# akvas/grates

Measured on AMD Instinct MI355X. Metric: d/o-96 solutions/s to 0.25deg grid + full-cov GFLOP/s at 1/2/4/8 MI355X, higher is better.
Workload: dtype f64; 1 GPU; batch of 240 monthly solutions d/o 96 -> 0.25 deg GeographicGrid (720x1440), kernel ewh, per GPU; max_degree=96, epochs_per_gpu=240, parallelism=epochs sharded over 1 GPU(s), no collective, fused_kernel=True, fourfold_symmetry=True, rotation_folded_kernel=True, rotations=10, settle_launches=300

## Files before the change

### grates_amd/_lib.py

```python

import ctypes
import os

_HERE = os.path.dirname(os.path.abspath(__file__))
LIB_PATH = os.path.join(_HERE, 'lib', 'libshg.so')

c_double_p = ctypes.c_void_p
c_plan_p = ctypes.c_void_p


class ShgError(RuntimeError):

    def __init__(self, function, status, message):
        super().__init__('{0} failed with status {1}: {2}'.format(function, status, message))
        self.function = function
        self.status = status


_POINTS_AT_TAIL = [ctypes.c_void_p, ctypes.c_void_p, ctypes.c_int, c_double_p, ctypes.c_int, ctypes.c_double, ctypes.c_double, c_double_p,
                   ctypes.c_void_p]

PROTOTYPES = {
    'shg_plan_create': [ctypes.POINTER(c_plan_p), ctypes.c_int, ctypes.c_int, c_double_p, c_double_p, ctypes.c_int, c_double_p, ctypes.c_int],
    'shg_plan_destroy': [c_plan_p],
    'shg_plan_set_chunk': [c_plan_p, ctypes.c_int],
    'shg_plan_set_path': [c_plan_p, ctypes.c_int],
    'shg_plan_set_rotations': [c_plan_p, ctypes.c_int],
    'shg_plan_set_stage_limit': [c_plan_p, ctypes.c_int],
    'shg_plan_set_order_pruning': [c_plan_p, ctypes.c_int],
    'shg_plan_order_cutoffs': [c_plan_p, ctypes.POINTER(ctypes.c_int), ctypes.c_int, ctypes.POINTER(ctypes.c_int), ctypes.POINTER(ctypes.c_int)],
    'shg_rot_order_cutoffs': [ctypes.c_int, ctypes.c_int, c_double_p, c_double_p, ctypes.POINTER(ctypes.c_int), ctypes.c_int, ctypes.POINTER(ctypes.c_int)],
    'shg_rot_level_tables': [ctypes.c_int, ctypes.c_int, ctypes.c_int, ctypes.c_int, ctypes.c_int, c_double_p, ctypes.POINTER(ctypes.c_int32), c_double_p,
                             ctypes.c_int64, ctypes.POINTER(ctypes.c_int32), ctypes.c_int64],
    'shg_plan_info': [c_plan_p, ctypes.POINTER(ctypes.c_int64)],
    'shg_analysis_info': [c_plan_p, c_double_p],
    'shg_plan_profile': [c_plan_p, ctypes.c_int],
    'shg_plan_profile_read': [c_plan_p, ctypes.POINTER(ctypes.c_double), ctypes.POINTER(ctypes.c_int64)],
    'shg_synthesis': [c_plan_p, c_double_p, ctypes.c_int, c_double_p, ctypes.c_void_p],
    'shg_synthesis_points': [ctypes.c_int, c_double_p, c_double_p, c_double_p, ctypes.c_int, c_double_p, ctypes.c_int, c_double_p, ctypes.c_void_p],
    'shg_legendre': [ctypes.c_int, c_double_p, ctypes.c_int, c_double_p, ctypes.c_void_p],
    'shg_legendre_order': [ctypes.c_int, ctypes.c_int, c_double_p, ctypes.c_int, c_double_p, ctypes.c_void_p],
    'shg_trigonometric': [ctypes.c_int, c_double_p, ctypes.c_int, c_double_p, ctypes.c_void_p],
    'shg_synthesis_matrix_order': [ctypes.c_int, ctypes.c_int, ctypes.c_int, c_double_p, ctypes.c_int, c_double_p, ctypes.c_int, c_double_p, ctypes.c_int,
                                   c_double_p, c_double_p, ctypes.c_void_p],
# ... 166 lines not shown
```

### grates_amd/csrc/common.h

```cpp
#pragma once

#include <hip/hip_runtime.h>

#include <algorithm>
#include <atomic>
#include <cstdarg>
#include <cstdint>
#include <cstdio>
#include <cstdlib>
#include <mutex>
#include <vector>

#include "../../include/shg.h"

namespace shg {

typedef double double4_t __attribute__((ext_vector_type(4)));

int fail(int code, const char* fmt, ...);
unsigned hip_failures();
int zero_fill(double* p, long long ld, long long cols, long long rows, hipStream_t stream);
int zero_fill(int* p, hipStream_t stream);
int triangle_copy(int n, const double* src, int ld, long long stride, int batch, double* dst, bool upper, hipStream_t stream);
enum ScratchSlot { kScratchSplitK = 0, kScratchAnaFold = 1, kScratchAnaTransform = 2, kScratchAnaSolution = 3, kScratchAnaFlag = 4,
// ... 210 lines not shown
constexpr int kRotPruneMaxDegree = 128;
constexpr int kEpochTile = 8;
constexpr int kLatTile = 64;

}

struct shg_plan {
    int device = 0;
    int N = 0, nlat = 0, nlon = 0;
    int ldlat = 0;
    bool sym4 = false;
    int rotR = 0;
    std::vector<double> lon_host;
    shg::DeviceArray<double> rot_trig;
    bool order_pruning = true;
    std::vector<int> rot_levels;
    std::vector<int> rot_level_set;
    std::vector<int> rot_trig_piece;
    std::vector<int> rot_item_rec, rot_item_nrec, rot_item_ntrip;
    shg::DeviceArray<int> rot_levtab_d;
    bool rot_levtab_valid = false;
    bool sym_ns = false;
    int ngroups = 1;
    int goff[5] = {0, 0, 0, 0, 0};
    int K = 0;
    int ncol = 0;
    int ncoltiles = 0;
    int chunk = 16;

    shg::DeviceArray<double> ct;
// ... 71 lines not shown
namespace shg {
int plan_alloc_workspace(shg_plan* p);
int fused_chunk_for(const shg_plan* p);
int build_pk_table(shg_plan* p, hipStream_t stream);
int build_pkf_table(shg_plan* p, bool ns, int rotR, hipStream_t stream);
int build_blockmap(shg_plan* p, int nbt, int nit, hipStream_t stream);
int pack_coefficients_fused(shg_plan* p, bool ns, int rotR, const double* anm, int B, hipStream_t stream);
int synthesis_fused(shg_plan* p, const double* anm, int B, double* grid, hipStream_t stream);
bool has_rotation_symmetry(int nlon, const double* lon, int R);
int rot_layout(int R, int N, int nk[kRotMaxClasses], int cnt[kRotMaxClasses], std::vector<int>* order_slot);
int rot_choose(int nlon, const double* lon_h, int N);
int rot_applicable(const shg_plan* p);
int build_rot_trig(shg_plan* p, const double* lon_h);
void rot_order_cutoffs(int N, int nlat, const double* colat, const double* kn, bool ns, std::vector<int>& levels);
std::vector<int> rot_level_list(int N, const std::vector<int>& levels);
void rot_trig_stream(int R, int N, int level, int nlon, const double* lon_h, std::vector<double>& tab);
void item_table_host(const shg_plan* p, int N, int level, int od, const std::vector<int>& qoff, int rotR, std::vector<int>& table, int& nrec, int& ntrip);
int synthesis_rot(shg_plan* p, const double* anm, int B, double* grid, hipStream_t stream);
int rot_kernel_waves();
int rot_set_stage_limit(shg_plan* p, int limit);
int fused32_applicable(const shg_plan* p);
int synthesis_fused32(shg_plan* p, const double* anm, int B, double* grid, hipStream_t stream);

struct PlanGuard {
    shg_plan* p;
    std::unique_lock<std::mutex> lock;
    PlanGuard(shg_plan* plan, hipStream_t stream) : p(plan), lock(plan->mtx) {
        if (p->used && p->last_stream != stream) {
            bool ordered = false;
            if (p->order_event || hipEventCreateWithFlags(&p->order_event, hipEventDisableTiming) == hipSuccess)
                ordered = hipEventRecord(p->order_event, p->last_stream) == hipSuccess && hipStreamWaitEvent(stream, p->order_event, 0) == hipSuccess;
// ... 19 lines not shown
```

### grates_amd/csrc/plan.hip

```cpp
#include <atomic>
#include <cmath>
#include <cstring>
#include <string>

#include <map>
#include <memory>
#include <mutex>
#include <utility>
#include <vector>

#include "common.h"

namespace shg {

static thread_local std::string g_last_error;
static std::atomic<unsigned> g_hip_failures{0};

int fail(int code, const char* fmt, ...) {
    char buf[512];
    va_list ap;
    va_start(ap, fmt);
    vsnprintf(buf, sizeof(buf), fmt, ap);
    va_end(ap);
    g_last_error = buf;
// ... 483 lines not shown

extern "C" int shg_plan_set_stage_limit(shg_plan* p, int limit) {
    SHG_REQUIRE(p != nullptr, "shg_plan_set_stage_limit: NULL plan");
    std::unique_lock<std::mutex> lock(p->mtx);
    return rot_set_stage_limit(p, limit);
}

extern "C" int shg_plan_set_order_pruning(shg_plan* p, int enable) {
    SHG_REQUIRE(p != nullptr, "shg_plan_set_order_pruning: NULL plan");
    SHG_REQUIRE(enable == 0 || enable == 1, "shg_plan_set_order_pruning: %d not in {0, 1}", enable);
    std::unique_lock<std::mutex> lock(p->mtx);
    p->order_pruning = enable != 0;
    return SHG_OK;
}

extern "C" int shg_plan_order_cutoffs(const shg_plan* p, int* levels, int capacity, int* nblocks, int* enabled) {
    SHG_REQUIRE(p != nullptr && nblocks != nullptr, "shg_plan_order_cutoffs: NULL argument");
    SHG_REQUIRE(capacity >= 0 && (levels != nullptr || capacity == 0), "shg_plan_order_cutoffs: NULL table of %d entries", capacity);
    const bool applies = rot_applicable(p) && !p->rot_levels.empty();
    *nblocks = applies ? (int)p->rot_levels.size() : 0;
    if (enabled) *enabled = applies && p->order_pruning ? 1 : 0;
    for (int i = 0; i < *nblocks && i < capacity; ++i) levels[i] = p->rot_levels[i];
    return SHG_OK;
}

extern "C" int shg_rot_order_cutoffs(int N, int nlat, const double* colat_h, const double* kn_h, int* levels, int capacity, int* nblocks) {
    SHG_REQUIRE(N >= 1 && N <= kRotPruneMaxDegree, "shg_rot_order_cutoffs: degree %d out of range [1, %d]", N, kRotPruneMaxDegree);
    SHG_REQUIRE(nlat > 0 && colat_h && kn_h && nblocks, "shg_rot_order_cutoffs: NULL or empty table");
    SHG_REQUIRE(capacity >= 0 && (levels != nullptr || capacity == 0), "shg_rot_order_cutoffs: NULL table of %d entries", capacity);
    std::vector<int> badmap, lv;
// ... 9 lines not shown
extern "C" int shg_rot_level_tables(int R, int N, int level, int ns, int nlon, const double* lon_h, int32_t header[24], double* trig, int64_t trig_capacity,
                                    int32_t* items, int64_t items_capacity) {
    SHG_REQUIRE(R == 3 || R == 6 || R == 9 || R == 10, "shg_rot_level_tables: %d rotations not in {3, 6, 9, 10}", R);
    SHG_REQUIRE(N >= 1 && N <= kRotPruneMaxDegree && level >= 1 && level <= N, "shg_rot_level_tables: level %d of degree %d out of range", level, N);
    SHG_REQUIRE(nlon >= 2 * R && nlon % (2 * R) == 0 && lon_h && header, "shg_rot_level_tables: NULL table or nlon %d no multiple of %d", nlon, 2 * R);
    SHG_REQUIRE(trig_capacity >= 0 && items_capacity >= 0 && (trig || trig_capacity == 0) && (items || items_capacity == 0), "shg_rot_level_tables: NULL table");
    for (int i = 0; i < kRotLevelInts; ++i) header[i] = 0;
    int nk[kRotMaxClasses], cnt[kRotMaxClasses];
    header[1] = rot_layout(R, level, nk, cnt, nullptr);
    header[0] = header[1] / 4;
    for (int c = 0; c < kRotMaxClasses; ++c) {
        header[8 + c] = nk[c];
        header[8 + kRotMaxClasses + c] = cnt[c];
    }
    std::vector<double> tab;
    rot_trig_stream(R, N, level, nlon, lon_h, tab);
    const int od = ns ? 16 : 8;
    std::vector<int> qoff(N + 2), table;
    int q = 0;
    for (int m = 0; m <= N; ++m) {
        qoff[m] = q;
        q += (N + 1 - m + od - 1) / od;
    }
    qoff[N + 1] = q;
    int nrec = 0, ntrip = 0;
    item_table_host(nullptr, N, level, od, qoff, R, table, nrec, ntrip);
    header[2] = nrec;
    header[3] = ntrip;
    header[4] = (int32_t)(tab.size() / 128);
    header[5] = (int32_t)(table.size() / 4);
    for (size_t i = 0; i < tab.size() && (int64_t)i < trig_capacity; ++i) trig[i] = tab[i];
// ... 15 lines not shown
        return fail(SHG_ERR_UNSUPPORTED, "shg_plan_set_rotations: the panel of %d rotations at degree %d does not fit the LDS", want, p->N);
    }
    SHG_HIP(hipDeviceSynchronize());
    if (rot_applicable(p)) {
        const int rc = build_rot_trig(p, p->lon_host.data());
        if (rc) return rc;
    }
    return SHG_OK;
}

extern "C" int shg_plan_info(const shg_plan* p, int64_t which[8]) {
    SHG_REQUIRE(p != nullptr && which != nullptr, "shg_plan_info: NULL argument");
    which[0] = p->N;
    which[1] = p->nlat;
    which[2] = p->nlon;
    which[3] = (p->sym4 ? 1 : 0) | (p->sym_ns ? 2 : 0) | (rot_applicable(p) ? 4 : 0);
    which[4] = p->chunk;
    which[5] = p->K;
    which[6] = (p->path >= 2 || (p->path == 0 && (rot_applicable(p) || fused_chunk_for(p) != 0 || fused32_applicable(p)))) ? 1 : 0;
    which[7] = p->path | (rot_applicable(p) ? p->rotR << 8 : 0);
    return SHG_OK;
}
```

### grates_amd/csrc/synthesis_rot.hip

```cpp
#include <algorithm>
#include <cmath>
#include <cstdlib>

#include "common.h"

#ifndef SHG_STORE_AUX
#define SHG_STORE_AUX 2
#endif

namespace shg {

typedef double double2_t __attribute__((ext_vector_type(2)));
typedef unsigned int uint4_t __attribute__((ext_vector_type(4)));

#ifndef SHG_ROT_PREFERENCE
#define SHG_ROT_PREFERENCE 10, 9, 6, 3
#endif
#ifndef SHG_ROT_WAVES
#define SHG_ROT_WAVES 8
#endif
#ifndef SHG_RING_DEPTH
#define SHG_RING_DEPTH (SHG_ROT_WAVES > 8 ? 3 : 5)
#endif
constexpr int kWaves = SHG_ROT_WAVES;
constexpr int kColStride = kWaves / 4;
constexpr int kRingDepth = SHG_RING_DEPTH;
constexpr int kRingSlots = kRingDepth + 1;
constexpr int kRingDoubles = kWaves * kRingSlots * 128;
constexpr int kMaxClasses = kRotMaxClasses;

template <int R>
struct RotTraits {
    static constexpr int kClasses = R / 2 + 1, kTwo = R % 2 == 0 ? 2 : 1, kAcc = 2 * R;
    static constexpr int acc_of(int r) { return r == 0 ? 0 : (R % 2 == 0 && 2 * r == R) ? 2 : 2 * kTwo + 4 * (r - 1); }
};

struct RotParams {
    int N, nlat, nlon, B, nit, nh;
    int nd;
    int nct;
    int npieces;
    int cls_nk[kMaxClasses];
    int cls_cnt[kMaxClasses];
    int nslot;
#ifdef SHG_EXPERIMENT
    int dbg;
    int stagger;
    int stagger2;
#endif
    int Qtot;
    const double* cpk4;
    const double* pkf;
    const int4* itemtab;
    int nrec, ntrip;
    int* tickets;
// ... 37 lines not shown

__device__ __forceinline__ void store_b64_soff(double v, int4_s rsrc, unsigned voff, unsigned soff) {
    asm volatile("s_mov_b32 m0, %3\n\ts_nop 0\n\tbuffer_store_dwordx2 %0, %1, %2, m0 offen nt"
                 :
                 : "v"(v), "v"(voff), "s"(rsrc), "s"(soff)
                 : "memory");
}

template <int N>
__device__ __forceinline__ void wait_vmcnt() {
    asm volatile("s_waitcnt vmcnt(%0)" ::"i"(N) : "memory");
    __builtin_amdgcn_sched_barrier(0);
}

template <int R>
__device__ __forceinline__ void rot_images(double4_t* acc, int r);

template <>
__device__ __forceinline__ void rot_images<6>(double4_t* acc, int r) {
    constexpr double g = 0.86602540378443864676;
    const double ca0 = acc[0][r], sb0 = acc[1][r], ca3 = acc[2][r], sb3 = acc[3][r];
    const double ca1 = acc[4][r], sa1 = acc[5][r], cb1 = acc[6][r], sb1 = acc[7][r];
    const double ca2 = acc[8][r], sa2 = acc[9][r], cb2 = acc[10][r], sb2 = acc[11][r];
#pragma unroll
    for (int sgn = 0; sgn < 2; ++sgn) {
        const double x0 = sgn ? ca0 - sb0 : ca0 + sb0, x3 = sgn ? ca3 - sb3 : ca3 + sb3;
        const double x1 = sgn ? ca1 - sb1 : ca1 + sb1, y1 = sgn ? cb1 + sa1 : cb1 - sa1;
        const double x2 = sgn ? ca2 - sb2 : ca2 + sb2, y2 = sgn ? cb2 + sa2 : cb2 - sa2;
        const double t = fma(-0.5, x2, x0);
        const double e0 = x0 + x2, e1 = fma(g, y2, t), e2 = fma(-g, y2, t);
        const double u = fma(0.5, x1, -x3);
        const double o0 = x1 + x3, o1 = fma(g, y1, u), o2 = fma(g, y1, -u);
        acc[6 * sgn + 0][r] = e0 + o0;
        acc[6 * sgn + 3][r] = e0 - o0;
        acc[6 * sgn + 1][r] = e1 + o1;
        acc[6 * sgn + 4][r] = e1 - o1;
        acc[6 * sgn + 2][r] = e2 + o2;
        acc[6 * sgn + 5][r] = e2 - o2;
    }
}

template <>
__device__ __forceinline__ void rot_images<3>(double4_t* acc, int r) {
    constexpr double g = 0.86602540378443864676;
    const double ca0 = acc[0][r], sb0 = acc[1][r];
    const double ca1 = acc[2][r], sa1 = acc[3][r], cb1 = acc[4][r], sb1 = acc[5][r];
#pragma unroll
    for (int sgn = 0; sgn < 2; ++sgn) {
        const double x0 = sgn ? ca0 - sb0 : ca0 + sb0;
        const double x1 = sgn ? ca1 - sb1 : ca1 + sb1, y1 = sgn ? cb1 + sa1 : cb1 - sa1;
        const double t = fma(-0.5, x1, x0);
        acc[3 * sgn + 0][r] = x0 + x1;
        acc[3 * sgn + 1][r] = fma(g, y1, t);
        acc[3 * sgn + 2][r] = fma(-g, y1, t);
    }
}

template <>
__device__ __forceinline__ void rot_images<9>(double4_t* acc, int r) {
    constexpr double c1 = 0.76604444311897803520, c2 = 0.17364817766693034885, c4 = -0.93969262078590838405;
    constexpr double s1 = 0.64278760968653932632, s2 = 0.98480775301220805937, s3 = 0.86602540378443864676, s4 = 0.34202014332566873304;
    const double ca0 = acc[0][r], sb0 = acc[1][r];
    double ca[4], sa[4], cb[4], sb[4];
#pragma unroll
    for (int j = 0; j < 4; ++j) {
        ca[j] = acc[2 + 4 * j][r];
        sa[j] = acc[3 + 4 * j][r];
        cb[j] = acc[4 + 4 * j][r];
        sb[j] = acc[5 + 4 * j][r];
    }
#pragma unroll
    for (int sgn = 0; sgn < 2; ++sgn) {
        const double x0 = sgn ? ca0 - sb0 : ca0 + sb0;
        double x[4], y[4];
#pragma unroll
        for (int j = 0; j < 4; ++j) {
            x[j] = sgn ? ca[j] - sb[j] : ca[j] + sb[j];
            y[j] = sgn ? cb[j] + sa[j] : cb[j] - sa[j];
        }
        const double x1 = x[0], x2 = x[1], x3 = x[2], x4 = x[3], y1 = y[0], y2 = y[1], y3 = y[2], y4 = y[3];
        const double t = (x1 + x2) + x4, x03 = x0 + x3;
        const double h = fma(-0.5, x3, x0), u = s3 * y3;
        const double C1 = fma(c1, x1, fma(c2, x2, fma(c4, x4, h)));
        const double C2 = fma(c2, x1, fma(c4, x2, fma(c1, x4, h)));
        const double C3 = fma(-0.5, t, x03);
        const double C4 = fma(c4, x1, fma(c1, x2, fma(c2, x4, h)));
        const double S1 = fma(s1, y1, fma(s2, y2, fma(s4, y4, u)));
        const double S2 = fma(s2, y1, fma(s4, y2, fma(-s1, y4, -u)));
        const double S3 = s3 * ((y1 - y2) + y4);
        const double S4 = fma(s4, y1, fma(-s1, y2, fma(-s2, y4, u)));
        acc[9 * sgn + 0][r] = x03 + t;
        acc[9 * sgn + 1][r] = C1 + S1;
        acc[9 * sgn + 8][r] = C1 - S1;
        acc[9 * sgn + 2][r] = C2 + S2;
        acc[9 * sgn + 7][r] = C2 - S2;
        acc[9 * sgn + 3][r] = C3 + S3;
        acc[9 * sgn + 6][r] = C3 - S3;
        acc[9 * sgn + 4][r] = C4 + S4;
        acc[9 * sgn + 5][r] = C4 - S4;
    }
}

template <>
__device__ __forceinline__ void rot_images<10>(double4_t* acc, int r) {
    constexpr double c1 = 0.80901699437494742410, c2 = 0.30901699437494742410;
    constexpr double s1 = 0.58778525229247312917, s2 = 0.95105651629515357212;
    const double ca0 = acc[0][r], sb0 = acc[1][r], ca5 = acc[2][r], sb5 = acc[3][r];
    double ca[4], sa[4], cb[4], sb[4];
#pragma unroll
    for (int j = 0; j < 4; ++j) {
        ca[j] = acc[4 + 4 * j][r];
        sa[j] = acc[5 + 4 * j][r];
        cb[j] = acc[6 + 4 * j][r];
        sb[j] = acc[7 + 4 * j][r];
    }
#pragma unroll
    for (int sgn = 0; sgn < 2; ++sgn) {
        const double x0 = sgn ? ca0 - sb0 : ca0 + sb0, x5 = sgn ? ca5 - sb5 : ca5 + sb5;
        double x[4], y[4];
#pragma unroll
        for (int j = 0; j < 4; ++j) {
            x[j] = sgn ? ca[j] - sb[j] : ca[j] + sb[j];
            y[j] = sgn ? cb[j] + sa[j] : cb[j] - sa[j];
        }
        const double x1 = x[0], x2 = x[1], x3 = x[2], x4 = x[3], y1 = y[0], y2 = y[1], y3 = y[2], y4 = y[3];
        const double e0 = (x0 + x2) + x4;
        const double a1 = fma(c2, x2, fma(-c1, x4, x0)), b1 = fma(s2, y2, s1 * y4);
        const double a2 = fma(-c1, x2, fma(c2, x4, x0)), b2 = fma(s1, y2, -(s2 * y4));
        const double e1 = a1 + b1, e4 = a1 - b1, e2 = a2 + b2, e3 = a2 - b2;
        const double o0 = (x1 + x3) + x5;
        const double p = fma(c1, x1, fma(-c2, x3, -x5)), q = fma(s1, y1, s2 * y3);
        const double u = fma(c2, x1, fma(-c1, x3, x5)), v = fma(s2, y1, -(s1 * y3));
        const double o1 = q + p, o4 = q - p, o2 = v + u, o3 = v - u;
        acc[10 * sgn + 0][r] = e0 + o0;
        acc[10 * sgn + 5][r] = e0 - o0;
        acc[10 * sgn + 1][r] = e1 + o1;
        acc[10 * sgn + 6][r] = e1 - o1;
        acc[10 * sgn + 2][r] = e2 + o2;
        acc[10 * sgn + 7][r] = e2 - o2;
        acc[10 * sgn + 3][r] = e3 + o3;
        acc[10 * sgn + 8][r] = e3 - o3;
        acc[10 * sgn + 4][r] = e4 + o4;
        acc[10 * sgn + 9][r] = e4 - o4;
    }
}

struct RotStream {
    const double* iptr;
    const double* ibase;
    const double* ifirst;
    const double* ilast;
    int irem;
    unsigned im0, ring_lds;
    int cslot, pf;
    double2_t tx, abx;
};

constexpr int EP = 4;
__device__ __forceinline__ void rot_stream_init(RotStream& S, const RotParams& P, const double* As, int wave) {
// ... 19 lines not shown
    return;
#endif
    S.im0 = S.im0 + 1024 == S.ring_lds + kRingSlots * 1024 ? S.ring_lds : S.im0 + 1024;
    const bool more = S.irem > 1;
    const double* nbase = S.ibase == S.ilast ? S.ifirst : S.ibase + kColStride * P.npieces * 128;
    S.ibase = more ? S.ibase : nbase;
    S.iptr = more ? S.iptr + 128 : nbase;
    S.irem = more ? S.irem - 1 : P.npieces;
}

template <bool NS, int R>
__device__ __forceinline__ void rot_phase2(const RotParams& P, const double* As, const double2_t* panel, RotStream& S, int wave, int lane,
                                           int b0, int it) {
    constexpr int PR = 16 * EP;
    using T = RotTraits<R>;
    constexpr int kImages = 2 * R;
    const int fr = lane & 15, fk = lane >> 4;
    const int i0 = it * 16, i0n = it * 8;
    const unsigned lane_off = (unsigned)lane * 16u;
    auto grid_row = [&](int s) { return NS ? (s < 8 ? i0n + s : P.nlat - 1 - (i0n + s - 8)) : i0 + s; };
    auto slot_valid = [&](int s) { return NS ? i0n + (s & 7) < P.nh : i0 + s < P.nlat; };

    const int grid_bytes = P.nlat * P.nlon * 8;
    const int n2 = P.nlon >> 1, nR = P.nlon / R;
    const double2_t* const ringp = reinterpret_cast<const double2_t*>(As) + wave * (kRingSlots * 64) + lane;
    const int rt = wave % EP;
    const double2_t* const prow = panel + rt * 16 + fr + fk * PR;
#define ROT_FETCH(T_, AB_)                                                                                \
    do {                                                                                                  \
        __builtin_amdgcn_sched_barrier(0);                                                                \
        if (!(SHG_ROT_X & 8)) rot_issue_piece(S, P, lane_off);                                            \
// ... 73 lines not shown
        {
            const double2_t* z = panel + P.nslot * PR + rt * 16 + fk;
#pragma unroll
            for (int r = 0; r < 4; ++r) acc[0][r] = z[4 * r].x;
        }
#pragma unroll
        for (int c = 0; c < T::kClasses; ++c) {
            if (c < T::kTwo) {
                ROT_CLASS(c, ROT_MFMA2, 2 * c, 2)
            } else {
                ROT_CLASS(c, ROT_MFMA4, 2 * T::kTwo + 4 * (c - T::kTwo), 4)
            }
        }
        ROT_STAMP(3 + 2 * min(q, 3));

#pragma unroll
        for (int r = 0; r < 4; ++r) rot_images<R>(acc, r);
        const int b = b0 + rt;
        const bool epoch_ok = b < P.B && !SHG_DBG(P, 1);
        double* const Gb = P.G + (size_t)min(b, P.B - 1) * P.nlat * P.nlon;
        {
            const __amdgpu_buffer_rsrc_t rsrc = __builtin_amdgcn_make_buffer_rsrc(Gb, 0, grid_bytes, 0x00020000);
            const int par = fr & 1, ce = fr & ~1;
            const int sa = fk + (par ? 8 : 0), sb = sa + 4;
            const bool col_ok = epoch_ok && ct * 16 + ce < P.nd;
            const unsigned row_a = col_ok && slot_valid(sa) ? (unsigned)grid_row(sa) * (unsigned)P.nlon * 8u : 0x80000000u;
            const unsigned row_b = col_ok && slot_valid(sb) ? (unsigned)grid_row(sb) * (unsigned)P.nlon * 8u : 0x80000000u;
            const unsigned asc = (unsigned)ce * 8u, desc = (unsigned)(14 - ce) * 8u;
#pragma unroll
            for (int t = 0; t < kImages; ++t) {
                const int k = t < R ? t : t - R;
                const bool ascending = t < R;
                int w = n2 + k * nR - (ascending ? 0 : P.nd);
                w = w >= P.nlon ? w - P.nlon : w;
                const int soff = (ascending ? w + 16 * ct : w + P.nd - 16 * ct - 16) * 8;
                double a_lo, a_hi, b_lo, b_hi;
                pair_exchange(acc[t][0], acc[t][2], 0xAAAAAAAAAAAAAAAAull, a_lo, a_hi);
                pair_exchange(acc[t][1], acc[t][3], 0xAAAAAAAAAAAAAAAAull, b_lo, b_hi);
                const double2_t va = ascending ? (double2_t){a_lo, a_hi} : (double2_t){a_hi, a_lo};
                const double2_t vb = ascending ? (double2_t){b_lo, b_hi} : (double2_t){b_hi, b_lo};
                const unsigned lane_col = (ascending ? asc : desc) + (unsigned)soff;
                __builtin_amdgcn_raw_buffer_store_b128(__builtin_bit_cast(uint4_t, va), rsrc, row_a + lane_col, 0, SHG_STORE_AUX);
                __builtin_amdgcn_raw_buffer_store_b128(__builtin_bit_cast(uint4_t, vb), rsrc, row_b + lane_col, 0, SHG_STORE_AUX);
            }
        }
        ROT_STAMP(4 + 2 * min(q, 3));
    }
    S.tx = tx;
    S.abx = abx;
#undef ROT_CLASS
#undef ROT_MFMA2
#undef ROT_MFMA4
#undef ROT_MFMA2_FIRST
#undef ROT_MFMA4_FIRST
#undef ROT_FETCH
}

__device__ __forceinline__ void panel_put(double2_t* panel, int index, double2_t v) { panel[index] = v; }
// ... 202 lines not shown
    if (P.stagger2 > 0 && wave >= EP) {
        const long long t0 = wall_clock64();
        for (int i = 0; i < 100000 && (long long)wall_clock64() - t0 < P.stagger2; ++i) __builtin_amdgcn_s_sleep(4);
    }
#endif

    if (wave / EP < P.nct && !SHG_DBG(P, 4)) {
        const double2_t* const ringp = reinterpret_cast<const double2_t*>(As) + wave * (kRingSlots * 64) + lane;
        rot_issue_piece(S, P, (unsigned)lane * 16u);
        wait_vmcnt<kRingDepth>();
        S.tx = ringp[0];
        S.cslot = 1;
        S.abx = panel[(wave % EP) * 16 + fr + fk * PR];
        S.pf = P.npieces > 1 ? 1 : 0;
        rot_phase2<NS, R>(P, As, panel, S, wave, lane, bt * 4, it);
        wait_vmcnt<4 * R>();
    } else {
        wait_vmcnt<0>();
    }
    ROT_STAMP(12);
}



static inline void order_class(int R, int m, int& cls, int& sign) {
    const int rho = m % R;
    const int r = 2 * rho <= R ? rho : R - rho;
    sign = 2 * rho <= R ? 1 : -1;
    if (R % 2 == 0)
        cls = r == 0 ? 0 : 2 * r == R ? 1 : r + 1;
    else
// ... 64 lines not shown
    if ((long long)p->nlat * p->nlon * 8 >= (1LL << 31)) return 0;
    return rot_fits(p->rotR, p->N) ? 1 : 0;
}

int rot_choose(int nlon, const double* lon_h, int N) {
    static const int kRotPreference[] = {SHG_ROT_PREFERENCE};
    int fallback = 0;
    for (int R : kRotPreference)
        if (has_rotation_symmetry(nlon, lon_h, R)) {
            if (N < 1 || rot_fits(R, N)) return R;
            if (!fallback) fallback = R;
        }
    return fallback;
}

void rot_trig_stream(int R, int N, int level, int nlon, const double* lon_h, std::vector<double>& tab) {
    (void)N;
    const int nd = nlon / (2 * R), nct = ceil_div(nd, 16);
    int nk[kMaxClasses], cnt[kMaxClasses];
    std::vector<int> order_slot;
    const int nslot = rot_layout(R, level, nk, cnt, &order_slot);
    const int npieces = nslot / 4;
    std::vector<int> slot_order(nslot, -1);
    for (int m = 1; m <= level; ++m) slot_order[order_slot[m]] = m;
    tab.assign(((size_t)nct * npieces + 1) * 128, 0.0);
    for (int ct = 0; ct < nct; ++ct)
        for (int ks = 0; ks < npieces; ++ks)
            for (int l = 0; l < 64; ++l) {
                const int m = slot_order[4 * ks + (l >> 4)], c = 16 * ct + (l & 15);
                if (m < 0 || c >= nd) continue;
                int cls, sg;
                order_class(R, m, cls, sg);
                const double arg = (double)m * lon_h[nlon / 2 + c];
                double* dst = &tab[(((size_t)ct * npieces + ks) * 64 + l) * 2];
                dst[0] = std::cos(arg);
                dst[1] = sg * std::sin(arg);
            }
}

int build_rot_trig(shg_plan* p, const double* lon_h) {
    const std::vector<int> full(1, p->N);
    const std::vector<int>& levels = p->rot_level_set.empty() ? full : p->rot_level_set;
    std::vector<double> all, tab;
    p->rot_trig_piece.clear();
    for (int level : levels) {
        rot_trig_stream(p->rotR, p->N, level, p->nlon, lon_h, tab);
        p->rot_trig_piece.push_back((int)(all.size() / 128));
        all.insert(all.end(), tab.begin(), tab.end());
    }
    p->rot_levtab_valid = false;
    return upload(p->rot_trig, all);
}

constexpr double kRotPruneTau = 1e-30;
constexpr int kRotLevelStep = 10;

void rot_order_cutoffs(int N, int nlat, const double* colat, const double* kn, bool ns, std::vector<int>& levels) {
    const int nh = nlat / 2;
    const int nit = ns ? ceil_div(nh, 8) : ceil_div(nlat, 16);
    levels.assign(nit, 0);
    std::vector<double> a, b, big(N + 1);
// ... 116 lines not shown
    int rc = build_pkf_table(p, ns, R, stream);
    if (rc) return rc;
    const int nbt = ceil_div(B, 4);
    const int nit = ns ? ceil_div(p->nlat / 2, 8) : ceil_div(p->nlat, 16);
    rc = pack_coefficients_fused(p, ns, R, anm, B, stream);
    if (rc) return rc;
    RotParams P;
    P.N = p->N;
    P.nlat = p->nlat;
    P.nlon = p->nlon;
    P.B = B;
    P.nit = nit;
    P.nh = p->nlat / 2;
    P.nd = p->nlon / (2 * R);
    P.nct = ceil_div(P.nd, 16);
    P.nslot = rot_layout(R, p->N, P.cls_nk, P.cls_cnt, nullptr);
    P.npieces = P.nslot / 4;
#ifdef SHG_EXPERIMENT
    P.dbg = experiment_switches();
    P.stagger = getenv("SHG_STAGGER") ? atoi(getenv("SHG_STAGGER")) : 0;
    P.stagger2 = getenv("SHG_STAGGER2") ? atoi(getenv("SHG_STAGGER2")) : 0;
#endif
    P.Qtot = p->Qtot;
    P.cpk4 = p->cpk4.get();
    P.pkf = p->pkf.get();
    P.itemtab = reinterpret_cast<const int4*>(p->itemtab_d.get());
    P.nrec = p->itemtab_nrec;
    P.ntrip = p->itemtab_ntrip;
    int limit = p->stage_limit;
    if (!p->stage_limit_set) {
// ... 60 lines not shown
```

### grates_amd/engine.py

```python

import collections
import ctypes
import hashlib

import numpy as np

from . import _lib


def _torch():
    import torch
    return torch


def require_gpu():
    torch = _torch()
    if not torch.cuda.is_available():
        raise RuntimeError('grates_amd: no GPU visible -- the hot path runs on MI355X only (there is no CPU fallback)')
    _lib.load()
    return torch


def device(index=None):
    torch = require_gpu()
# ... 46 lines not shown
        if handle is not None and handle.value:
            try:
                _lib.load().shg_plan_destroy(handle)
            except Exception:
                pass
            self._handle = None

    def info(self):
        arr = (ctypes.c_int64 * 8)()
        _lib.call('shg_plan_info', self._handle, arr)
        nblocks, enabled = ctypes.c_int(0), ctypes.c_int(0)
        _lib.call('shg_plan_order_cutoffs', self._handle, None, 0, ctypes.byref(nblocks), ctypes.byref(enabled))
        levels = (ctypes.c_int * max(nblocks.value, 1))()
        _lib.call('shg_plan_order_cutoffs', self._handle, levels, nblocks.value, ctypes.byref(nblocks), ctypes.byref(enabled))
        return {'max_degree': arr[0], 'nlat': arr[1], 'nlon': arr[2], 'fourfold_symmetry': bool(arr[3] & 1), 'north_south_symmetry': bool(arr[3] & 2),
                'rotation_symmetry': bool(arr[3] & 4), 'epochs_per_pass': arr[4], 'k_slots': arr[5], 'fused': bool(arr[6]), 'path': int(arr[7]) & 0xff, 'rotations': int(arr[7]) >> 8,
                'order_pruning': bool(enabled.value), 'order_cutoffs': [int(levels[i]) for i in range(nblocks.value)]}

    def set_path(self, path):
        _lib.call('shg_plan_set_path', self._handle, {'auto': 0, 'staged': 1, 'fused': 2, 'fused32': 5, 'rot': 6}[path])

    def set_stage_limit(self, limit):
        _lib.call('shg_plan_set_stage_limit', self._handle, int(limit))

    def set_order_pruning(self, enable):
        _lib.call('shg_plan_set_order_pruning', self._handle, 1 if enable else 0)

    def set_rotations(self, R):
        _lib.call('shg_plan_set_rotations', self._handle, int(R))

    def set_chunk(self, epochs_per_pass):
        _lib.call('shg_plan_set_chunk', self._handle, int(epochs_per_pass))

    PROFILE_KINDS = ('pack_coefficients', 'legendre_stage', 'lon_stage', 'covprop', 'analysis_lon', 'analysis_solve', 'k6', 'k7')

    def profile(self, enable=True, kinds=None):
        if enable and kinds:
            mask = 0
            for name in kinds:
                mask |= 1 << (self.PROFILE_KINDS.index(name) + 1)
            _lib.call('shg_plan_profile', self._handle, mask)
# ... 1634 lines not shown
```

### include/shg.h

```cpp
#ifndef SHG_H
#define SHG_H

#include <stdint.h>

#ifdef __cplusplus
extern "C" {
#endif

typedef struct shg_plan shg_plan;

typedef enum {
    SHG_OK = 0,
    SHG_ERR_INVALID = -1,
    SHG_ERR_HIP = -2,
    SHG_ERR_NOMEM = -3,
    SHG_ERR_UNSUPPORTED = -4
} shg_status;

int shg_plan_create(shg_plan** out, int N, int nlat, const double* colat_h, const double* kn_h,
                    int nlon, const double* lon_h, int device);
int shg_plan_destroy(shg_plan* plan);

int shg_plan_set_chunk(shg_plan* plan, int epochs_per_pass);

int shg_plan_set_path(shg_plan* plan, int path);

int shg_plan_set_stage_limit(shg_plan* plan, int limit);

int shg_plan_set_rotations(shg_plan* plan, int R);

int shg_plan_set_order_pruning(shg_plan* plan, int enable);
int shg_plan_order_cutoffs(const shg_plan* plan, int* levels, int capacity, int* nblocks, int* enabled);
int shg_rot_order_cutoffs(int N, int nlat, const double* colat_h, const double* kn_h, int* levels, int capacity, int* nblocks);
int shg_rot_level_tables(int R, int N, int level, int ns, int nlon, const double* lon_h, int32_t header[24], double* trig,
                         int64_t trig_capacity, int32_t* items, int64_t items_capacity);

int shg_plan_info(const shg_plan* plan, int64_t which[8]);

#define SHG_PROFILE_KINDS 8
int shg_plan_profile(shg_plan* plan, int enable);
int shg_plan_profile_read(shg_plan* plan, double ms[SHG_PROFILE_KINDS], int64_t launches[SHG_PROFILE_KINDS]);

int shg_synthesis(shg_plan* plan, const double* anm, int B, double* grid, void* stream);

int shg_synthesis_points(int N, const double* colat, const double* lon, const double* kn, int npts,
                         const double* anm, int B, double* values, void* stream);

int shg_epoch_rms(const double* values, int B, long long M, int accumulate, long long count, double* acc, void* stream);

int shg_legendre(int N, const double* colat, int k, double* pnm, void* stream);
// ... 209 lines not shown
```

Measured before the change: 510,300 solutions/s.

## Fold half-filled last column tile by mirroring columns into padding lanes

When the per-rotation column count leaves the last 16-wide tile half full, the padding lanes now get trig values for the mirrored (descending) columns. That tile then computes only the ascending images, which also cover the mirror half. This removes the second butterfly and the descending stores for that tile, and the kernel waits on fewer outstanding stores. The butterfly code is restructured into a split step plus per-sign halves, with wrap handling for odd rotation counts. The fold uses long-double trig and changes the store addressing, so it risks subtle indexing errors.

```diff
diff --git a/grates_amd/_lib.py b/grates_amd/_lib.py
--- a/grates_amd/_lib.py
+++ b/grates_amd/_lib.py
@@ -28,6 +28,7 @@
     'shg_plan_set_rotations': [c_plan_p, ctypes.c_int],
     'shg_plan_set_stage_limit': [c_plan_p, ctypes.c_int],
     'shg_plan_set_order_pruning': [c_plan_p, ctypes.c_int],
+    'shg_plan_set_half_tile_fold': [c_plan_p, ctypes.c_int],
     'shg_plan_order_cutoffs': [c_plan_p, ctypes.POINTER(ctypes.c_int), ctypes.c_int, ctypes.POINTER(ctypes.c_int), ctypes.POINTER(ctypes.c_int)],
     'shg_rot_order_cutoffs': [ctypes.c_int, ctypes.c_int, c_double_p, c_double_p, ctypes.POINTER(ctypes.c_int), ctypes.c_int, ctypes.POINTER(ctypes.c_int)],
     'shg_rot_level_tables': [ctypes.c_int, ctypes.c_int, ctypes.c_int, ctypes.c_int, ctypes.c_int, c_double_p, ctypes.POINTER(ctypes.c_int32), c_double_p,
diff --git a/grates_amd/csrc/common.h b/grates_amd/csrc/common.h
--- a/grates_amd/csrc/common.h
+++ b/grates_amd/csrc/common.h
@@ -248,6 +248,7 @@
     std::vector<double> lon_host;
     shg::DeviceArray<double> rot_trig;
     bool order_pruning = true;
+    bool half_tile_fold = true;
     std::vector<int> rot_levels;
     std::vector<int> rot_level_set;
     std::vector<int> rot_trig_piece;
@@ -349,7 +350,7 @@
 int build_rot_trig(shg_plan* p, const double* lon_h);
 void rot_order_cutoffs(int N, int nlat, const double* colat, const double* kn, bool ns, std::vector<int>& levels);
 std::vector<int> rot_level_list(int N, const std::vector<int>& levels);
-void rot_trig_stream(int R, int N, int level, int nlon, const double* lon_h, std::vector<double>& tab);
+void rot_trig_stream(int R, int N, int level, int nlon, const double* lon_h, std::vector<double>& tab, bool fill_half);
 void item_table_host(const shg_plan* p, int N, int level, int od, const std::vector<int>& qoff, int rotR, std::vector<int>& table, int& nrec, int& ntrip);
 int synthesis_rot(shg_plan* p, const double* anm, int B, double* grid, hipStream_t stream);
 int rot_kernel_waves();
diff --git a/grates_amd/csrc/plan.hip b/grates_amd/csrc/plan.hip
--- a/grates_amd/csrc/plan.hip
+++ b/grates_amd/csrc/plan.hip
@@ -521,6 +521,14 @@
     return SHG_OK;
 }
 
+extern "C" int shg_plan_set_half_tile_fold(shg_plan* p, int enable) {
+    SHG_REQUIRE(p != nullptr, "shg_plan_set_half_tile_fold: NULL plan");
+    SHG_REQUIRE(enable == 0 || enable == 1, "shg_plan_set_half_tile_fold: %d not in {0, 1}", enable);
+    std::unique_lock<std::mutex> lock(p->mtx);
+    p->half_tile_fold = enable != 0;
+    return SHG_OK;
+}
+
 extern "C" int shg_plan_order_cutoffs(const shg_plan* p, int* levels, int capacity, int* nblocks, int* enabled) {
     SHG_REQUIRE(p != nullptr && nblocks != nullptr, "shg_plan_order_cutoffs: NULL argument");
     SHG_REQUIRE(capacity >= 0 && (levels != nullptr || capacity == 0), "shg_plan_order_cutoffs: NULL table of %d entries", capacity);
@@ -560,7 +568,7 @@
         header[8 + kRotMaxClasses + c] = cnt[c];
     }
     std::vector<double> tab;
-    rot_trig_stream(R, N, level, nlon, lon_h, tab);
+    rot_trig_stream(R, N, level, nlon, lon_h, tab, false);
     const int od = ns ? 16 : 8;
     std::vector<int> qoff(N + 2), table;
     int q = 0;
@@ -606,7 +614,8 @@
     which[0] = p->N;
     which[1] = p->nlat;
     which[2] = p->nlon;
-    which[3] = (p->sym4 ? 1 : 0) | (p->sym_ns ? 2 : 0) | (rot_applicable(p) ? 4 : 0);
+    which[3] = (p->sym4 ? 1 : 0) | (p->sym_ns ? 2 : 0) | (rot_applicable(p) ? 4 : 0) |
+               (rot_applicable(p) && p->half_tile_fold && (p->nlon / (2 * p->rotR)) % 16 == 8 ? 8 : 0);
     which[4] = p->chunk;
     which[5] = p->K;
     which[6] = (p->path >= 2 || (p->path == 0 && (rot_applicable(p) || fused_chunk_for(p) != 0 || fused32_applicable(p)))) ? 1 : 0;
diff --git a/grates_amd/csrc/synthesis_rot.hip b/grates_amd/csrc/synthesis_rot.hip
--- a/grates_amd/csrc/synthesis_rot.hip
+++ b/grates_amd/csrc/synthesis_rot.hip
@@ -33,12 +33,17 @@
 struct RotTraits {
     static constexpr int kClasses = R / 2 + 1, kTwo = R % 2 == 0 ? 2 : 1, kAcc = 2 * R;
     static constexpr int acc_of(int r) { return r == 0 ? 0 : (R % 2 == 0 && 2 * r == R) ? 2 : 2 * kTwo + 4 * (r - 1); }
+    static constexpr bool two_sums(int r) { return r == 0 || 2 * r == R; }
+    static constexpr int x_of(int r, int s) { return acc_of(r) + (two_sums(r) ? s : 3 * s); }
+    static constexpr int y_of(int r, int s) { return two_sums(r) ? -1 : acc_of(r) + 2 - s; }
+    static constexpr int img_of(int k, int s) { return k < kTwo ? x_of(k == 0 ? 0 : R / 2, s) : (k - kTwo) % 2 == 0 ? x_of(1 + (k - kTwo) / 2, s) : y_of(1 + (k - kTwo) / 2, s); }
 };
 
 struct RotParams {
     int N, nlat, nlon, B, nit, nh;
     int nd;
     int nct;
+    int half_fold;
     int npieces;
     int cls_nk[kMaxClasses];
     int cls_cnt[kMaxClasses];
@@ -106,135 +111,120 @@
 }
 
 template <int R>
-__device__ __forceinline__ void rot_images(double4_t* acc, int r);
-
-template <>
-__device__ __forceinline__ void rot_images<6>(double4_t* acc, int r) {
+__device__ __forceinline__ void rot_split(double4_t* acc, int r) {
+    using T = RotTraits<R>;
+#pragma unroll
+    for (int c = 0; c <= R / 2; ++c) {
+        const int a = T::acc_of(c);
+        if (T::two_sums(c)) {
+            const double ca = acc[a][r], sb = acc[a + 1][r];
+            acc[T::x_of(c, 0)][r] = ca + sb;
+            acc[T::x_of(c, 1)][r] = ca - sb;
+        } else {
+            const double ca = acc[a][r], sa = acc[a + 1][r], cb = acc[a + 2][r], sb = acc[a + 3][r];
+            acc[T::x_of(c, 0)][r] = ca + sb;
+            acc[T::y_of(c, 0)][r] = cb - sa;
+            acc[T::x_of(c, 1)][r] = ca - sb;
+            acc[T::y_of(c, 1)][r] = cb + sa;
+        }
+    }
+}
+
+template <int S>
+__device__ __forceinline__ void rot_half6(double4_t* acc, int r) {
+    using T = RotTraits<6>;
     constexpr double g = 0.86602540378443864676;
-    const double ca0 = acc[0][r], sb0 = acc[1][r], ca3 = acc[2][r], sb3 = acc[3][r];
-    const double ca1 = acc[4][r], sa1 = acc[5][r], cb1 = acc[6][r], sb1 = acc[7][r];
-    const double ca2 = acc[8][r], sa2 = acc[9][r], cb2 = acc[10][r], sb2 = acc[11][r];
-#pragma unroll
-    for (int sgn = 0; sgn < 2; ++sgn) {
-        const double x0 = sgn ? ca0 - sb0 : ca0 + sb0, x3 = sgn ? ca3 - sb3 : ca3 + sb3;
-        const double x1 = sgn ? ca1 - sb1 : ca1 + sb1, y1 = sgn ? cb1 + sa1 : cb1 - sa1;
-        const double x2 = sgn ? ca2 - sb2 : ca2 + sb2, y2 = sgn ? cb2 + sa2 : cb2 - sa2;
-        const double t = fma(-0.5, x2, x0);
-        const double e0 = x0 + x2, e1 = fma(g, y2, t), e2 = fma(-g, y2, t);
-        const double u = fma(0.5, x1, -x3);
-        const double o0 = x1 + x3, o1 = fma(g, y1, u), o2 = fma(g, y1, -u);
-        acc[6 * sgn + 0][r] = e0 + o0;
-        acc[6 * sgn + 3][r] = e0 - o0;
-        acc[6 * sgn + 1][r] = e1 + o1;
-        acc[6 * sgn + 4][r] = e1 - o1;
-        acc[6 * sgn + 2][r] = e2 + o2;
-        acc[6 * sgn + 5][r] = e2 - o2;
-    }
-}
-
-template <>
-__device__ __forceinline__ void rot_images<3>(double4_t* acc, int r) {
+    const double x0 = acc[T::x_of(0, S)][r], x3 = acc[T::x_of(3, S)][r];
+    const double x1 = acc[T::x_of(1, S)][r], y1 = acc[T::y_of(1, S)][r];
+    const double x2 = acc[T::x_of(2, S)][r], y2 = acc[T::y_of(2, S)][r];
+    const double t = fma(-0.5, x2, x0);
+    const double e0 = x0 + x2, e1 = fma(g, y2, t), e2 = fma(-g, y2, t);
+    const double u = fma(0.5, x1, -x3);
+    const double o0 = x1 + x3, o1 = fma(g, y1, u), o2 = fma(g, y1, -u);
+    acc[T::img_of(0, S)][r] = e0 + o0;
+    acc[T::img_of(3, S)][r] = e0 - o0;
+    acc[T::img_of(1, S)][r] = e1 + o1;
+    acc[T::img_of(4, S)][r] = e1 - o1;
+    acc[T::img_of(2, S)][r] = e2 + o2;
+    acc[T::img_of(5, S)][r] = e2 - o2;
+}
+
+template <int S>
+__device__ __forceinline__ void rot_half3(double4_t* acc, int r) {
+    using T = RotTraits<3>;
     constexpr double g = 0.86602540378443864676;
-    const double ca0 = acc[0][r], sb0 = acc[1][r];
-    const double ca1 = acc[2][r], sa1 = acc[3][r], cb1 = acc[4][r], sb1 = acc[5][r];
-#pragma unroll
-    for (int sgn = 0; sgn < 2; ++sgn) {
-        const double x0 = sgn ? ca0 - sb0 : ca0 + sb0;
-        const double x1 = sgn ? ca1 - sb1 : ca1 + sb1, y1 = sgn ? cb1 + sa1 : cb1 - sa1;
-        const double t = fma(-0.5, x1, x0);
-        acc[3 * sgn + 0][r] = x0 + x1;
-        acc[3 * sgn + 1][r] = fma(g, y1, t);
-        acc[3 * sgn + 2][r] = fma(-g, y1, t);
-    }
-}
-
-template <>
-__device__ __forceinline__ void rot_images<9>(double4_t* acc, int r) {
+    const double x0 = acc[T::x_of(0, S)][r];
+    const double x1 = acc[T::x_of(1, S)][r], y1 = acc[T::y_of(1, S)][r];
+    const double t = fma(-0.5, x1, x0);
+    acc[T::img_of(0, S)][r] = x0 + x1;
+    acc[T::img_of(1, S)][r] = fma(g, y1, t);
+    acc[T::img_of(2, S)][r] = fma(-g, y1, t);
+}
+
+template <int S>
+__device__ __forceinline__ void rot_half9(double4_t* acc, int r) {
+    using T = RotTraits<9>;
     constexpr double c1 = 0.76604444311897803520, c2 = 0.17364817766693034885, c4 = -0.93969262078590838405;
     constexpr double s1 = 0.64278760968653932632, s2 = 0.98480775301220805937, s3 = 0.86602540378443864676, s4 = 0.34202014332566873304;
-    const double ca0 = acc[0][r], sb0 = acc[1][r];
-    double ca[4], sa[4], cb[4], sb[4];
-#pragma unroll
-    for (int j = 0; j < 4; ++j) {
-        ca[j] = acc[2 + 4 * j][r];
-        sa[j] = acc[3 + 4 * j][r];
-        cb[j] = acc[4 + 4 * j][r];
-        sb[j] = acc[5 + 4 * j][r];
-    }
-#pragma unroll
-    for (int sgn = 0; sgn < 2; ++sgn) {
-        const double x0 = sgn ? ca0 - sb0 : ca0 + sb0;
-        double x[4], y[4];
-#pragma unroll
-        for (int j = 0; j < 4; ++j) {
-            x[j] = sgn ? ca[j] - sb[j] : ca[j] + sb[j];
-            y[j] = sgn ? cb[j] + sa[j] : cb[j] - sa[j];
-        }
-        const double x1 = x[0], x2 = x[1], x3 = x[2], x4 = x[3], y1 = y[0], y2 = y[1], y3 = y[2], y4 = y[3];
-        const double t = (x1 + x2) + x4, x03 = x0 + x3;
-        const double h = fma(-0.5, x3, x0), u = s3 * y3;
-        const double C1 = fma(c1, x1, fma(c2, x2, fma(c4, x4, h)));
-        const double C2 = fma(c2, x1, fma(c4, x2, fma(c1, x4, h)));
-        const double C3 = fma(-0.5, t, x03);
-        const double C4 = fma(c4, x1, fma(c1, x2, fma(c2, x4, h)));
-        const double S1 = fma(s1, y1, fma(s2, y2, fma(s4, y4, u)));
-        const double S2 = fma(s2, y1, fma(s4, y2, fma(-s1, y4, -u)));
-        const double S3 = s3 * ((y1 - y2) + y4);
-        const double S4 = fma(s4, y1, fma(-s1, y2, fma(-s2, y4, u)));
-        acc[9 * sgn + 0][r] = x03 + t;
-        acc[9 * sgn + 1][r] = C1 + S1;
-        acc[9 * sgn + 8][r] = C1 - S1;
-        acc[9 * sgn + 2][r] = C2 + S2;
-        acc[9 * sgn + 7][r] = C2 - S2;
-        acc[9 * sgn + 3][r] = C3 + S3;
-        acc[9 * sgn + 6][r] = C3 - S3;
-        acc[9 * sgn + 4][r] = C4 + S4;
-        acc[9 * sgn + 5][r] = C4 - S4;
-    }
-}
-
-template <>
-__device__ __forceinline__ void rot_images<10>(double4_t* acc, int r) {
+    const double x0 = acc[T::x_of(0, S)][r];
+    const double x1 = acc[T::x_of(1, S)][r], x2 = acc[T::x_of(2, S)][r], x3 = acc[T::x_of(3, S)][r], x4 = acc[T::x_of(4, S)][r];
+    const double y1 = acc[T::y_of(1, S)][r], y2 = acc[T::y_of(2, S)][r], y3 = acc[T::y_of(3, S)][r], y4 = acc[T::y_of(4, S)][r];
+    const double t = (x1 + x2) + x4, x03 = x0 + x3;
+    const double h = fma(-0.5, x3, x0), u = s3 * y3;
+    const double C1 = fma(c1, x1, fma(c2, x2, fma(c4, x4, h)));
+    const double C2 = fma(c2, x1, fma(c4, x2, fma(c1, x4, h)));
+    const double C3 = fma(-0.5, t, x03);
+    const double C4 = fma(c4, x1, fma(c1, x2, fma(c2, x4, h)));
+    const double S1 = fma(s1, y1, fma(s2, y2, fma(s4, y4, u)));
+    const double S2 = fma(s2, y1, fma(s4, y2, fma(-s1, y4, -u)));
+    const double S3 = s3 * ((y1 - y2) + y4);
+    const double S4 = fma(s4, y1, fma(-s1, y2, fma(-s2, y4, u)));
+    acc[T::img_of(0, S)][r] = x03 + t;
+    acc[T::img_of(1, S)][r] = C1 + S1;
+    acc[T::img_of(8, S)][r] = C1 - S1;
+    acc[T::img_of(2, S)][r] = C2 + S2;
+    acc[T::img_of(7, S)][r] = C2 - S2;
+    acc[T::img_of(3, S)][r] = C3 + S3;
+    acc[T::img_of(6, S)][r] = C3 - S3;
+    acc[T::img_of(4, S)][r] = C4 + S4;
+    acc[T::img_of(5, S)][r] = C4 - S4;
+}
+
+template <int S>
+__device__ __forceinline__ void rot_half10(double4_t* acc, int r) {
+    using T = RotTraits<10>;
     constexpr double c1 = 0.80901699437494742410, c2 = 0.30901699437494742410;
     constexpr double s1 = 0.58778525229247312917, s2 = 0.95105651629515357212;
-    const double ca0 = acc[0][r], sb0 = acc[1][r], ca5 = acc[2][r], sb5 = acc[3][r];
-    double ca[4], sa[4], cb[4], sb[4];
-#pragma unroll
-    for (int j = 0; j < 4; ++j) {
-        ca[j] = acc[4 + 4 * j][r];
-        sa[j] = acc[5 + 4 * j][r];
-        cb[j] = acc[6 + 4 * j][r];
-        sb[j] = acc[7 + 4 * j][r];
-    }
-#pragma unroll
-    for (int sgn = 0; sgn < 2; ++sgn) {
-        const double x0 = sgn ? ca0 - sb0 : ca0 + sb0, x5 = sgn ? ca5 - sb5 : ca5 + sb5;
-        double x[4], y[4];
-#pragma unroll
-        for (int j = 0; j < 4; ++j) {
-            x[j] = sgn ? ca[j] - sb[j] : ca[j] + sb[j];
-            y[j] = sgn ? cb[j] + sa[j] : cb[j] - sa[j];
-        }
-        const double x1 = x[0], x2 = x[1], x3 = x[2], x4 = x[3], y1 = y[0], y2 = y[1], y3 = y[2], y4 = y[3];
-        const double e0 = (x0 + x2) + x4;
-        const double a1 = fma(c2, x2, fma(-c1, x4, x0)), b1 = fma(s2, y2, s1 * y4);
-        const double a2 = fma(-c1, x2, fma(c2, x4, x0)), b2 = fma(s1, y2, -(s2 * y4));
-        const double e1 = a1 + b1, e4 = a1 - b1, e2 = a2 + b2, e3 = a2 - b2;
-        const double o0 = (x1 + x3) + x5;
-        const double p = fma(c1, x1, fma(-c2, x3, -x5)), q = fma(s1, y1, s2 * y3);
-        const double u = fma(c2, x1, fma(-c1, x3, x5)), v = fma(s2, y1, -(s1 * y3));
-        const double o1 = q + p, o4 = q - p, o2 = v + u, o3 = v - u;
-        acc[10 * sgn + 0][r] = e0 + o0;
-        acc[10 * sgn + 5][r] = e0 - o0;
-        acc[10 * sgn + 1][r] = e1 + o1;
-        acc[10 * sgn + 6][r] = e1 - o1;
-        acc[10 * sgn + 2][r] = e2 + o2;
-        acc[10 * sgn + 7][r] = e2 - o2;
-        acc[10 * sgn + 3][r] = e3 + o3;
-        acc[10 * sgn + 8][r] = e3 - o3;
-        acc[10 * sgn + 4][r] = e4 + o4;
-        acc[10 * sgn + 9][r] = e4 - o4;
-    }
+    const double x0 = acc[T::x_of(0, S)][r], x5 = acc[T::x_of(5, S)][r];
+    const double x1 = acc[T::x_of(1, S)][r], x2 = acc[T::x_of(2, S)][r], x3 = acc[T::x_of(3, S)][r], x4 = acc[T::x_of(4, S)][r];
+    const double y1 = acc[T::y_of(1, S)][r], y2 = acc[T::y_of(2, S)][r], y3 = acc[T::y_of(3, S)][r], y4 = acc[T::y_of(4, S)][r];
+    const double e0 = (x0 + x2) + x4;
+    const double a1 = fma(c2, x2, fma(-c1, x4, x0)), b1 = fma(s2, y2, s1 * y4);
+    const double a2 = fma(-c1, x2, fma(c2, x4, x0)), b2 = fma(s1, y2, -(s2 * y4));
+    const double e1 = a1 + b1, e4 = a1 - b1, e2 = a2 + b2, e3 = a2 - b2;
+    const double o0 = (x1 + x3) + x5;
+    const double p = fma(c1, x1, fma(-c2, x3, -x5)), q = fma(s1, y1, s2 * y3);
+    const double u = fma(c2, x1, fma(-c1, x3, x5)), v = fma(s2, y1, -(s1 * y3));
+    const double o1 = q + p, o4 = q - p, o2 = v + u, o3 = v - u;
+    acc[T::img_of(0, S)][r] = e0 + o0;
+    acc[T::img_of(5, S)][r] = e0 - o0;
+    acc[T::img_of(1, S)][r] = e1 + o1;
+    acc[T::img_of(6, S)][r] = e1 - o1;
+    acc[T::img_of(2, S)][r] = e2 + o2;
+    acc[T::img_of(7, S)][r] = e2 - o2;
+    acc[T::img_of(3, S)][r] = e3 + o3;
+    acc[T::img_of(8, S)][r] = e3 - o3;
+    acc[T::img_of(4, S)][r] = e4 + o4;
+    acc[T::img_of(9, S)][r] = e4 - o4;
+}
+
+template <int R, int S>
+__device__ __forceinline__ void rot_half(double4_t* acc, int r) {
+    static_assert(R == 10 || R == 9 || R == 6 || R == 3, "no butterfly for this rotation count");
+    if constexpr (R == 10) rot_half10<S>(acc, r);
+    else if constexpr (R == 9) rot_half9<S>(acc, r);
+    else if constexpr (R == 6) rot_half6<S>(acc, r);
+    else rot_half3<S>(acc, r);
 }
 
 struct RotStream {
@@ -284,7 +274,6 @@
                                            int b0, int it) {
     constexpr int PR = 16 * EP;
     using T = RotTraits<R>;
-    constexpr int kImages = 2 * R;
     const int fr = lane & 15, fk = lane >> 4;
     const int i0 = it * 16, i0n = it * 8;
     const unsigned lane_off = (unsigned)lane * 16u;
@@ -388,34 +377,49 @@
         }
         ROT_STAMP(3 + 2 * min(q, 3));
 
-#pragma unroll
-        for (int r = 0; r < 4; ++r) rot_images<R>(acc, r);
+        const bool fold = P.half_fold != 0 && ct == P.nct - 1;
         const int b = b0 + rt;
         const bool epoch_ok = b < P.B && !SHG_DBG(P, 1);
         double* const Gb = P.G + (size_t)min(b, P.B - 1) * P.nlat * P.nlon;
-        {
-            const __amdgpu_buffer_rsrc_t rsrc = __builtin_amdgcn_make_buffer_rsrc(Gb, 0, grid_bytes, 0x00020000);
-            const int par = fr & 1, ce = fr & ~1;
-            const int sa = fk + (par ? 8 : 0), sb = sa + 4;
-            const bool col_ok = epoch_ok && ct * 16 + ce < P.nd;
-            const unsigned row_a = col_ok && slot_valid(sa) ? (unsigned)grid_row(sa) * (unsigned)P.nlon * 8u : 0x80000000u;
-            const unsigned row_b = col_ok && slot_valid(sb) ? (unsigned)grid_row(sb) * (unsigned)P.nlon * 8u : 0x80000000u;
-            const unsigned asc = (unsigned)ce * 8u, desc = (unsigned)(14 - ce) * 8u;
+        const __amdgpu_buffer_rsrc_t rsrc = __builtin_amdgcn_make_buffer_rsrc(Gb, 0, grid_bytes, 0x00020000);
+        const int par = fr & 1, ce = fr & ~1;
+        const int sa = fk + (par ? 8 : 0), sb = sa + 4;
+        const bool col_ok = epoch_ok && ct * 16 + ce < (fold ? P.nd + 8 : P.nd);
+        const unsigned row_a = col_ok && slot_valid(sa) ? (unsigned)grid_row(sa) * (unsigned)P.nlon * 8u : 0x80000000u;
+        const unsigned row_b = col_ok && slot_valid(sb) ? (unsigned)grid_row(sb) * (unsigned)P.nlon * 8u : 0x80000000u;
+        const unsigned asc_a = row_a + (unsigned)ce * 8u, asc_b = row_b + (unsigned)ce * 8u;
+        const unsigned desc_a = row_a + (unsigned)(14 - ce) * 8u, desc_b = row_b + (unsigned)(14 - ce) * 8u;
+        auto put_image = [&](const double4_t& v, bool ascending, unsigned lane_a, unsigned lane_b, int soff) {
+            double a_lo, a_hi, b_lo, b_hi;
+            pair_exchange(v[0], v[2], 0xAAAAAAAAAAAAAAAAull, a_lo, a_hi);
+            pair_exchange(v[1], v[3], 0xAAAAAAAAAAAAAAAAull, b_lo, b_hi);
+            const double2_t va = ascending ? (double2_t){a_lo, a_hi} : (double2_t){a_hi, a_lo};
+            const double2_t vb = ascending ? (double2_t){b_lo, b_hi} : (double2_t){b_hi, b_lo};
+            __builtin_amdgcn_raw_buffer_store_b128(__builtin_bit_cast(uint4_t, va), rsrc, lane_a + (unsigned)soff, 0, SHG_STORE_AUX);
+            __builtin_amdgcn_raw_buffer_store_b128(__builtin_bit_cast(uint4_t, vb), rsrc, lane_b + (unsigned)soff, 0, SHG_STORE_AUX);
+        };
 #pragma unroll
-            for (int t = 0; t < kImages; ++t) {
-                const int k = t < R ? t : t - R;
-                const bool ascending = t < R;
-                int w = n2 + k * nR - (ascending ? 0 : P.nd);
-                w = w >= P.nlon ? w - P.nlon : w;
-                const int soff = (ascending ? w + 16 * ct : w + P.nd - 16 * ct - 16) * 8;
-                double a_lo, a_hi, b_lo, b_hi;
-                pair_exchange(acc[t][0], acc[t][2], 0xAAAAAAAAAAAAAAAAull, a_lo, a_hi);
-                pair_exchange(acc[t][1], acc[t][3], 0xAAAAAAAAAAAAAAAAull, b_lo, b_hi);
-                const double2_t va = ascending ? (double2_t){a_lo, a_hi} : (double2_t){a_hi, a_lo};
-                const double2_t vb = ascending ? (double2_t){b_lo, b_hi} : (double2_t){b_hi, b_lo};
-                const unsigned lane_col = (ascending ? asc : desc) + (unsigned)soff;
-                __builtin_amdgcn_raw_buffer_store_b128(__builtin_bit_cast(uint4_t, va), rsrc, row_a + lane_col, 0, SHG_STORE_AUX);
-                __builtin_amdgcn_raw_buffer_store_b128(__builtin_bit_cast(uint4_t, vb), rsrc, row_b + lane_col, 0, SHG_STORE_AUX);
+        for (int r = 0; r < 4; ++r) rot_split<R>(acc, r);
+#pragma unroll
+        for (int k = 0; k < R; ++k) asm volatile("" : "+v"(acc[T::img_of(k, 1)]));
+#pragma unroll
+        for (int r = 0; r < 4; ++r) rot_half<R, 0>(acc, r);
+        const unsigned row_wrap = R % 2 != 0 && ce >= 8 ? (unsigned)P.nlon * 8u : 0u;
+        int w = n2;
+#pragma unroll
+        for (int k = 0; k < R; ++k) {
+            const bool wraps = R % 2 != 0 && w + 16 * ct + 16 > P.nlon;
+            put_image(acc[T::img_of(k, 0)], true, wraps ? asc_a - row_wrap : asc_a, wraps ? asc_b - row_wrap : asc_b, (w + 16 * ct) * 8);
+            w = w + nR >= P.nlon ? w + nR - P.nlon : w + nR;
+        }
+        if (!fold) {
+#pragma unroll
+            for (int r = 0; r < 4; ++r) rot_half<R, 1>(acc, r);
+            w = n2 - P.nd;
+#pragma unroll
+            for (int k = 0; k < R; ++k) {
+                put_image(acc[T::img_of(k, 1)], false, desc_a, desc_b, (w + P.nd - 16 * ct - 16) * 8);
+                w = w + nR >= P.nlon ? w + nR - P.nlon : w + nR;
             }
         }
         ROT_STAMP(4 + 2 * min(q, 3));
@@ -648,7 +652,10 @@
         S.abx = panel[(wave % EP) * 16 + fr + fk * PR];
         S.pf = P.npieces > 1 ? 1 : 0;
         rot_phase2<NS, R>(P, As, panel, S, wave, lane, bt * 4, it);
-        wait_vmcnt<4 * R>();
+        if (P.half_fold != 0)
+            wait_vmcnt<2 * R>();
+        else
+            wait_vmcnt<4 * R>();
     } else {
         wait_vmcnt<0>();
     }
@@ -743,9 +750,10 @@
     return fallback;
 }
 
-void rot_trig_stream(int R, int N, int level, int nlon, const double* lon_h, std::vector<double>& tab) {
+void rot_trig_stream(int R, int N, int level, int nlon, const double* lon_h, std::vector<double>& tab, bool fill_half) {
     (void)N;
     const int nd = nlon / (2 * R), nct = ceil_div(nd, 16);
+    const long double pi = 3.141592653589793238462643383279502884L;
     int nk[kMaxClasses], cnt[kMaxClasses];
     std::vector<int> order_slot;
     const int nslot = rot_layout(R, level, nk, cnt, &order_slot);
@@ -757,13 +765,19 @@
         for (int ks = 0; ks < npieces; ++ks)
             for (int l = 0; l < 64; ++l) {
                 const int m = slot_order[4 * ks + (l >> 4)], c = 16 * ct + (l & 15);
-                if (m < 0 || c >= nd) continue;
+                if (m < 0 || (c >= nd && !(fill_half && nd % 16 == 8))) continue;
                 int cls, sg;
                 order_class(R, m, cls, sg);
-                const double arg = (double)m * lon_h[nlon / 2 + c];
                 double* dst = &tab[(((size_t)ct * npieces + ks) * 64 + l) * 2];
-                dst[0] = std::cos(arg);
-                dst[1] = sg * std::sin(arg);
+                if (c < nd) {
+                    const double arg = (double)m * lon_h[nlon / 2 + c];
+                    dst[0] = std::cos(arg);
+                    dst[1] = sg * std::sin(arg);
+                } else {
+                    const long double arg = (long double)m * (2 * pi / R - (long double)lon_h[nlon / 2 + 2 * nd - 1 - c]);
+                    dst[0] = (double)std::cos(arg);
+                    dst[1] = sg * (double)std::sin(arg);
+                }
             }
 }
 
@@ -773,7 +787,7 @@
     std::vector<double> all, tab;
     p->rot_trig_piece.clear();
     for (int level : levels) {
-        rot_trig_stream(p->rotR, p->N, level, p->nlon, lon_h, tab);
+        rot_trig_stream(p->rotR, p->N, level, p->nlon, lon_h, tab, true);
         p->rot_trig_piece.push_back((int)(all.size() / 128));
         all.insert(all.end(), tab.begin(), tab.end());
     }
@@ -920,6 +934,7 @@
     P.nh = p->nlat / 2;
     P.nd = p->nlon / (2 * R);
     P.nct = ceil_div(P.nd, 16);
+    P.half_fold = p->half_tile_fold && P.nd % 16 == 8 ? 1 : 0;
     P.nslot = rot_layout(R, p->N, P.cls_nk, P.cls_cnt, nullptr);
     P.npieces = P.nslot / 4;
 #ifdef SHG_EXPERIMENT
diff --git a/grates_amd/engine.py b/grates_amd/engine.py
--- a/grates_amd/engine.py
+++ b/grates_amd/engine.py
@@ -84,7 +84,7 @@
         levels = (ctypes.c_int * max(nblocks.value, 1))()
         _lib.call('shg_plan_order_cutoffs', self._handle, levels, nblocks.value, ctypes.byref(nblocks), ctypes.byref(enabled))
         return {'max_degree': arr[0], 'nlat': arr[1], 'nlon': arr[2], 'fourfold_symmetry': bool(arr[3] & 1), 'north_south_symmetry': bool(arr[3] & 2),
-                'rotation_symmetry': bool(arr[3] & 4), 'epochs_per_pass': arr[4], 'k_slots': arr[5], 'fused': bool(arr[6]), 'path': int(arr[7]) & 0xff, 'rotations': int(arr[7]) >> 8,
+                'rotation_symmetry': bool(arr[3] & 4), 'half_tile_fold': bool(arr[3] & 8), 'epochs_per_pass': arr[4], 'k_slots': arr[5], 'fused': bool(arr[6]), 'path': int(arr[7]) & 0xff, 'rotations': int(arr[7]) >> 8,
                 'order_pruning': bool(enabled.value), 'order_cutoffs': [int(levels[i]) for i in range(nblocks.value)]}
 
     def set_path(self, path):
@@ -95,6 +95,9 @@
 
     def set_order_pruning(self, enable):
         _lib.call('shg_plan_set_order_pruning', self._handle, 1 if enable else 0)
+
+    def set_half_tile_fold(self, enable):
+        _lib.call('shg_plan_set_half_tile_fold', self._handle, 1 if enable else 0)
 
     def set_rotations(self, R):
         _lib.call('shg_plan_set_rotations', self._handle, int(R))
diff --git a/include/shg.h b/include/shg.h
--- a/include/shg.h
+++ b/include/shg.h
@@ -34,6 +34,8 @@
 int shg_rot_order_cutoffs(int N, int nlat, const double* colat_h, const double* kn_h, int* levels, int capacity, int* nblocks);
 int shg_rot_level_tables(int R, int N, int level, int ns, int nlon, const double* lon_h, int32_t header[24], double* trig,
                          int64_t trig_capacity, int32_t* items, int64_t items_capacity);
+
+int shg_plan_set_half_tile_fold(shg_plan* plan, int enable);
 
 int shg_plan_info(const shg_plan* plan, int64_t which[8]);
 
```

Result: faster. 515,900 solutions/s, median of 6 (+1.1%).
